# debbiemarkslab/BEAR

Measured on AMD Instinct MI355X. Metric: k-mer contexts/sec (DM-marginal+grad h), k=13, higher is better.
Workload: dtype f64

## Files before the change

bear_amd/csrc/bear_cnn.hip:

```cpp
#include "bear_host.h"
#include "kernels_cnn.h"

int cnn_ws_setup(bear_ws *) { return allow_dynamic_lds({BEAR_KFN(cnn_backward_head_kernel)}, cnh_lds_bytes()); }

#ifdef CNN_STAMPS
extern "C" int bear_dbg_cnn_stamps(unsigned long long *host_out, int reset) {
  if (host_out) HIP_TRY(hipMemcpyFromSymbol(host_out, HIP_SYMBOL(cnn_stamp_sums), sizeof(unsigned long long) * 8));
  if (reset) {
    unsigned long long z[8] = {0, 0, 0, 0, 0, 0, 0, 0};
    HIP_TRY(hipMemcpyToSymbol(HIP_SYMBOL(cnn_stamp_sums), z, sizeof(z)));
  }
  return BEAR_OK;
}
#endif

static int cnn_forward_grid(const bear_ws *ws, uint64_t groups) {
  return grid_capped((groups + CNN_THREADS / 64 - 1) / (CNN_THREADS / 64), (uint64_t)ws->num_cu * 16);
}

static int cnn_check(const bear_ws *ws, int lag, int fw, int nf, int l1) {
  int st = check_ws(ws);
  if (st != BEAR_OK) return st;
  if (lag < 1 || lag > CNN_MAX_LAG || fw < 1 || fw > lag || nf != CNN_NF || l1 != CNN_L1) return BEAR_ERR_INVALID_ARG;
  return BEAR_OK;
// ... 13 lines not shown
  if (!kmer_code || !params || !prior || misaligned(t1_save) || misaligned8(prior)) return BEAR_ERR_INVALID_ARG;
  const cnn_dims D = cnn_make_dims(lag, filter_width);
  const size_t lds = sizeof(double) * (BEAR_EXPTAB_N + (size_t)filter_width * 6 * CNN_NF + (CNN_THREADS / 64) * CNN_FWD_SCRATCH);
  const int blocks = grid_capped((n_rows + CNN_THREADS - 1) / CNN_THREADS, (uint64_t)ws->num_cu * 16);
  hipLaunchKernelGGL(cnn_forward_kernel, dim3((unsigned)blocks), dim3(CNN_THREADS), lds, static_cast<hipStream_t>(stream),
                     reinterpret_cast<const unsigned long long *>(kmer_code), n_rows, D, params, prior, t1_save,
                     static_cast<const pln_tile *>(nullptr), static_cast<const uint16_t *>(nullptr), (n_rows + 63) / 64, cnn_all_positions(D));
  HIP_TRY(hipGetLastError());
  return BEAR_OK;
}

static int cnn_backward_grid(bear_ws *ws, const cnn_dims &D, uint64_t n_rows, int filter_width, int *waves_out, int *parts_out,
                             size_t *lds_out, uint64_t *blocks_out, hipStream_t s, int may_alloc) {
  const size_t fixed = sizeof(double) * (BEAR_EXPTAB_N + (size_t)filter_width * 6 * CNN_NF + (size_t)((D.total + 1) & ~1));
  const size_t lds2 = sizeof(double) * (cnnq_fixed_doubles(D) + (size_t)cnnq<2>::WAVES * cnnq<2>::WAVE_DOUBLES);
  const char *force = getenv("BEAR_CNN_BACKWARD");
  const bool det = bear_deterministic();
  int waves = det ? 1 : 4, parts = 0;
  while (waves > 1 && fixed + (size_t)waves * CNN_WAVE_DOUBLES * sizeof(double) > 160u * 1024u) waves >>= 1;
  size_t lds = fixed + (size_t)waves * CNN_WAVE_DOUBLES * sizeof(double);
  uint64_t per_block = (uint64_t)64 * waves;
  if (lds2 <= 160u * 1024u && !(force && force[0] == '1')) {
    parts = 1;
    waves = det ? 1 : cnnq<2>::WAVES;
    lds = sizeof(double) * (cnnq_fixed_doubles(D) + (size_t)waves * cnnq<2>::WAVE_DOUBLES);
    per_block = (uint64_t)cnnq<2>::TILE * waves;
  }
  if (lds > 160u * 1024u) return BEAR_ERR_INVALID_ARG;
  const uint64_t blocks = (uint64_t)grid_capped((n_rows + per_block - 1) / per_block, (uint64_t)ws->num_cu);
  const size_t need = (size_t)blocks * D.total;
  if (ws->cnn_partials_cap < need) {
    if (!may_alloc) return BEAR_ERR_INVALID_ARG;
    HIP_TRY(hipStreamSynchronize(s));
    if (ws->cnn_partials) (void)hipFree(ws->cnn_partials);
    ws->cnn_partials = nullptr;
    ws->cnn_partials_cap = 0;
    HIP_TRY(hipMalloc(&ws->cnn_partials, sizeof(double) * need));
    ws->cnn_partials_cap = need;
  }
  *waves_out = waves;
  *parts_out = parts;
  *lds_out = lds;
  *blocks_out = blocks;
  return BEAR_OK;
}

static int launch_cnn_backward(bear_ws *ws, const cnn_dims &D, const uint64_t *kmer_code, uint64_t n_rows, int filter_width,
                               const double *params, const double *t1_save, const double *prior, const double *grad_prior,
                               double *grad_params, hipStream_t s, int may_alloc, const bear_plan *live_plan = nullptr) {
  int waves = 0, parts = 0;
  size_t lds = 0;
  uint64_t blocks = 0;
  int st = cnn_backward_grid(ws, D, n_rows, filter_width, &waves, &parts, &lds, &blocks, s, may_alloc);
  if (st != BEAR_OK) return st;
  const bool parts2 = parts != 0;
  const void *fn = parts2 ? reinterpret_cast<const void *>(cnn_backward_parts_kernel<2>) : reinterpret_cast<const void *>(cnn_backward_kernel);
  if (may_alloc) HIP_TRY(hipFuncSetAttribute(fn, hipFuncAttributeMaxDynamicSharedMemorySize, (int)lds));
  const unsigned long long *kc = reinterpret_cast<const unsigned long long *>(kmer_code);
  if (parts2) {
    const bool lists = live_plan && live_plan->live && live_plan->n_live_rows < n_rows;
    const uint64_t groups = lists ? live_plan->n_tiles : (n_rows + cnnq<2>::TILE - 1) / cnnq<2>::TILE;
    hipLaunchKernelGGL(cnn_backward_parts_kernel<2>, dim3((unsigned)blocks), dim3(64 * waves), lds, s, kc, n_rows, D, params, t1_save, prior,
                       grad_prior, ws->cnn_partials, lists ? live_plan->tiles : nullptr, lists ? live_plan->live : nullptr, groups,
                       cnn_all_positions(D));
  }
  else
    hipLaunchKernelGGL(cnn_backward_kernel, dim3((unsigned)blocks), dim3(64 * waves), lds, s, kc, n_rows, D, params, t1_save, prior,
                       grad_prior, ws->cnn_partials);
  hipLaunchKernelGGL(cnn_finalize_kernel, dim3((D.total + 3) / 4), dim3(256), 0, s, ws->cnn_partials, (int)blocks, D.total, grad_params);
  HIP_TRY(hipGetLastError());
  return BEAR_OK;
}

int bear_cnn_backward_f64(bear_ws *ws, const uint64_t *kmer_code, uint64_t n_rows, int lag, int filter_width, int num_filters,
                          int layer1_width, const double *params, const double *t1_save, const double *prior,
                          const double *grad_prior, double *grad_params, void *stream) {
  int st = cnn_check(ws, lag, filter_width, num_filters, layer1_width);
  if (st != BEAR_OK) return st;
  if (!params || !grad_params) return BEAR_ERR_INVALID_ARG;
  if (n_rows && (!kmer_code || !t1_save || !prior || !grad_prior || misaligned(t1_save))) return BEAR_ERR_INVALID_ARG;
  const cnn_dims D = cnn_make_dims(lag, filter_width);
  return launch_cnn_backward(ws, D, kmer_code, n_rows, filter_width, params, t1_save, prior, grad_prior, grad_params,
                             static_cast<hipStream_t>(stream), 1);
}

int bear_cnn_reserve(bear_ws *ws, uint64_t n_rows, int lag, int filter_width, int num_filters, int layer1_width) {
  int st = cnn_check(ws, lag, filter_width, num_filters, layer1_width);
  if (st != BEAR_OK) return st;
  const cnn_dims D = cnn_make_dims(lag, filter_width);
  int waves = 0, parts = 0;
  size_t lds = 0;
  uint64_t blocks = 0;
  st = cnn_backward_grid(ws, D, n_rows, filter_width, &waves, &parts, &lds, &blocks, nullptr, 1);
  if (st != BEAR_OK) return st;
  HIP_TRY(hipFuncSetAttribute(parts ? reinterpret_cast<const void *>(cnn_backward_parts_kernel<2>)
                                                      : reinterpret_cast<const void *>(cnn_backward_kernel),
                              hipFuncAttributeMaxDynamicSharedMemorySize, (int)lds));
  return BEAR_OK;
}

static int cnn_forward_levels(bear_ws *ws, const bear_plan *plan, const cnn_dims &D, const uint64_t *kmer_code, uint64_t n_rows,
                              const double *params, double *prior, double *t1_buf, hipStream_t s);
static cnn_level_io cnn_level_positions(const bear_plan *plan, const cnn_dims &D, int k) {
  const int K = plan->n_cnn_levels;
  const int L = k == 0 ? D.lag : plan->cnn_levels[k - 1].letters;
  cnn_level_io io = cnn_all_positions(D);
  io.p_hi = L - D.fw + 1;
  io.p_lo = k == K ? 0 : plan->cnn_levels[k].letters - D.fw + 1;
  io.head = k == 0;
  io.p_hi -= plan->n_cnn_win[k];
  return io;
}
static cnn_level_io cnn_window_positions(const cnn_dims &D, const bear_window_dev &wt) {
  cnn_level_io io = cnn_all_positions(D);
  io.p_lo = wt.pos;
  io.p_hi = io.p_lo + 1;
  io.head = 0;
  return io;
}
static void cnn_level_sources(const bear_plan *plan, int k, cnn_level_io &io) {
  if (k < plan->n_cnn_levels) {
    io.t1_parent = plan->cnn_levels[k].rows;
    io.parent = plan->cnn_levels[k].parent_of_below;
  }
  io.n_win = plan->n_cnn_win[k];
  for (int q = 0; q < plan->n_cnn_win[k]; ++q) {
    io.win_rows[q] = plan->cnn_win[k][q].rows;
    io.win_row_of[q] = plan->cnn_win[k][q].row_of_context;
  }
}
static bool cnn_parts_form_forced_off() {
  const char *force = getenv("BEAR_CNN_BACKWARD");
  return force && force[0] == '1';
}
static int cnn_train_reduce_levels(bear_ws *ws, const bear_plan *plan, const cnn_dims &D, const uint64_t *kmer_code, uint64_t n_rows,
                                   const double *theta, double *prior_buf, double *t1_buf, double *grad_rows_buf, double eps, int train_ar,
                                   double *packed, hipStream_t s) {
  const int K = plan->n_cnn_levels;
  const double *params = theta + 1;
  int bw_waves = 0, bw_parts = 0;
  size_t bw_lds = 0;
  uint64_t bw_blocks = 0;
  int st = cnn_backward_grid(ws, D, n_rows, D.fw, &bw_waves, &bw_parts, &bw_lds, &bw_blocks, s, 0);
  if (st != BEAR_OK) return st;
  if (!bw_parts) return BEAR_ERR_INVALID_ARG;
  auto level_codes = [&](int k) { return k == 0 ? reinterpret_cast<const unsigned long long *>(kmer_code) : plan->cnn_levels[k - 1].codes; };
  auto level_rows = [&](int k) { return k == 0 ? n_rows : plan->cnn_levels[k - 1].n; };
  auto level_table = [&](int k) { return k == 0 ? t1_buf : plan->cnn_levels[k - 1].rows; };
  auto level_io = [&](int k) { return cnn_level_positions(plan, D, k); };
  const cnn_level_io io0 = level_io(0);
  const bool recompute_t1 = io0.p_lo >= io0.p_hi && !getenv("BEAR_AMD_CNN_KEEP_T1");
  st = cnn_forward_levels(ws, plan, D, kmer_code, n_rows, params, prior_buf, recompute_t1 ? nullptr : t1_buf, s);
  if (st != BEAR_OK) return st;
  st = launch_prior_plan_grad(ws, plan, prior_buf, params_eps(eps), theta, train_ar, 1, packed, grad_rows_buf, s);
  if (st != BEAR_OK) return st;
  const uint64_t per_block = (uint64_t)cnnq<2>::TILE * (uint64_t)bw_waves;
  bool first_launch = true;
  auto backward = [&](const unsigned long long *codes, uint64_t n, const double *t1_in, cnn_level_io io) {
    const uint64_t blocks = first_launch ? bw_blocks : (uint64_t)grid_capped((n + per_block - 1) / per_block, bw_blocks);
    io.accumulate = first_launch ? 0 : 1;
    first_launch = false;
    hipLaunchKernelGGL(cnn_backward_parts_kernel<2>, dim3((unsigned)blocks), dim3(64 * bw_waves), bw_lds, s, codes, n, D, params, t1_in, prior_buf,
                       grad_rows_buf, ws->cnn_partials, static_cast<const pln_tile *>(nullptr), static_cast<const uint16_t *>(nullptr),
                       (n + cnnq<2>::TILE - 1) / cnnq<2>::TILE, io);
  };
  for (int k = 0; k <= K; ++k) {
    cnn_level_io io = level_io(k);
    const uint64_t n = level_rows(k);
    const int W = plan->n_cnn_win[k];
    if (k > 0) {
      const int sb = grid_capped((n * (CNN_L1 / 2) + 255) / 256, (uint64_t)ws->num_cu * 32);
      hipLaunchKernelGGL(cnn_level_sum_kernel, dim3((unsigned)sb), dim3(256), 0, s, level_table(k - 1), plan->cnn_levels[k - 1].child_start,
                         n, level_table(k));
    }
    io.dT1 = (k == 0 && (K > 0 || W > 0)) ? t1_buf : (k > 0 ? level_table(k) : nullptr);
    if (k == 0 && recompute_t1) cnn_level_sources(plan, 0, io);
    if (k == 0 && io.p_lo >= io.p_hi && !getenv("BEAR_AMD_CNN_NO_HEAD_KERNEL")) {
      io.accumulate = first_launch ? 0 : 1;
      first_launch = false;
      hipLaunchKernelGGL(cnn_backward_head_kernel, dim3((unsigned)bw_blocks), dim3(CNH_WAVES * 64), cnh_lds_bytes(), s, n, D, params,
                         recompute_t1 ? static_cast<const double *>(nullptr) : t1_buf, prior_buf, grad_rows_buf, ws->cnn_partials, io);
    } else if (k == 0 || io.p_lo < io.p_hi) {
      backward(level_codes(k), n, (k == 0 && recompute_t1) ? static_cast<const double *>(nullptr) : t1_buf, io);
    }
    for (int q = 0; q < W; ++q) {
      const bear_window_dev &wt = plan->cnn_win[k][q];
      const int sb = grid_capped((wt.n + 3) / 4, (uint64_t)ws->num_cu * 8);
      hipLaunchKernelGGL(cnn_window_sum_kernel, dim3((unsigned)sb), dim3(256), 0, s, level_table(k), wt.perm, wt.child_start, wt.n, wt.rows);
      cnn_level_io wio = cnn_window_positions(D, wt);
      wio.dT1 = wt.rows;
      backward(wt.codes, wt.n, t1_buf, wio);
    }
  }
  hipLaunchKernelGGL(cnn_finalize_kernel, dim3((D.total + 3) / 4), dim3(256), 0, s, ws->cnn_partials, (int)bw_blocks, D.total, packed + 2);
  HIP_TRY(hipGetLastError());
  return BEAR_OK;
}

static void plan_drop_cnn_levels(bear_plan *plan) {
  for (int k = 0; k < plan->n_cnn_levels; ++k) {
    plan->bytes -= plan->cnn_levels[k].bytes;
    bear_level_free(&plan->cnn_levels[k]);
  }
  for (int k = 0; k <= CNN_MAX_LAG; ++k) {
    for (int q = 0; q < plan->n_cnn_win[k]; ++q) {
      plan->bytes -= plan->cnn_win[k][q].bytes;
      bear_window_free(&plan->cnn_win[k][q]);
    }
    plan->n_cnn_win[k] = 0;
  }
  plan->n_cnn_levels = 0;
  plan->n_cnn_windows = 0;
  plan->cnn_codes = nullptr;
}

int bear_plan_attach_cnn_levels(bear_plan *plan, const uint64_t *kmer_code, int lag, int filter_width, int *n_levels, void *stream) {
  if (n_levels) *n_levels = 0;
  if (!plan || plan->ncol != 5 || lag < 1 || lag > CNN_MAX_LAG || filter_width < 1 || filter_width > lag) return BEAR_ERR_INVALID_ARG;
  if (plan->n_rows && (!kmer_code || misaligned(kmer_code))) return BEAR_ERR_INVALID_ARG;
  hipStream_t s = static_cast<hipStream_t>(stream);
  HIP_TRY(hipStreamSynchronize(s));
  plan_drop_cnn_levels(plan);
  const cnn_dims D = cnn_make_dims(lag, filter_width);
  if (sizeof(double) * (cnnq_fixed_doubles(D) + (size_t)cnnq<2>::WAVES * cnnq<2>::WAVE_DOUBLES) > 160u * 1024u) return BEAR_OK;
  if (plan->n_rows < 2 || plan->n_live_rows != plan->n_rows) return BEAR_OK;
  const unsigned long long *below = reinterpret_cast<const unsigned long long *>(kmer_code);
  uint64_t n_below = plan->n_rows;
  int misses = 0;
  double keep_ratio = 0.6;
  if (const char *r = getenv("BEAR_AMD_CNN_LEVEL_RATIO")) keep_ratio = atof(r);
  for (int k = 1; k <= D.P - 1 && misses < 3; ++k) {
    bear_level_dev lv;
    const int st = bear_level_build(below, n_below, lag - k, &lv, s);
    if (st != BEAR_OK) {
      if (st == BEAR_ERR_HIP) g_last_hip_error = bear_count_last_hip_error();
      plan_drop_cnn_levels(plan);
      return st;
    }
    if ((double)lv.n > keep_ratio * (double)n_below) {
      bear_level_free(&lv);
      ++misses;
      continue;
    }
    misses = 0;
    lv.bytes = lv.n * (8 + 4 + 16 * 8) + 4 * n_below;
    plan->cnn_levels[plan->n_cnn_levels++] = lv;
    plan->bytes += lv.bytes;
    below = lv.codes;
    n_below = lv.n;
  }
  if (!getenv("BEAR_AMD_CNN_NO_WINDOWS")) {
    const int K = plan->n_cnn_levels;
    for (int k = 0; k <= K; ++k) {
      const unsigned long long *codes_k = k == 0 ? reinterpret_cast<const unsigned long long *>(kmer_code) : plan->cnn_levels[k - 1].codes;
      const uint64_t n_k = k == 0 ? plan->n_rows : plan->cnn_levels[k - 1].n;
      const int L = k == 0 ? lag : plan->cnn_levels[k - 1].letters;
      const int p_hi = L - filter_width + 1, p_lo = k == K ? 0 : plan->cnn_levels[k].letters - filter_width + 1;
      bear_window_dev built[CNN_MAX_WIN];
      int nb = 0;
      for (int p = p_hi - 1; p >= p_lo && nb < CNN_MAX_WIN && n_k >= 64; --p) {
        bear_window_dev wt;
        const int st = bear_window_build(codes_k, n_k, p, filter_width, &wt, s);
        if (st != BEAR_OK) {
          if (st == BEAR_ERR_HIP) g_last_hip_error = bear_count_last_hip_error();
          for (int q = 0; q < nb; ++q) bear_window_free(&built[q]);
          plan_drop_cnn_levels(plan);
          return st;
        }
        if (wt.n * 8 > n_k) {
          bear_window_free(&wt);
          break;
        }
        built[nb++] = wt;
      }
      for (int q = 0; q < nb; ++q) {
        plan->cnn_win[k][q] = built[nb - 1 - q];
        plan->bytes += plan->cnn_win[k][q].bytes;
      }
      plan->n_cnn_win[k] = nb;
      plan->n_cnn_windows += nb;
    }
  }
  if (plan->n_cnn_levels || plan->n_cnn_windows) {
    plan->cnn_codes = kmer_code;
    plan->cnn_lag = lag;
    plan->cnn_fw = filter_width;
  }
  if (n_levels) *n_levels = plan->n_cnn_levels;
  return BEAR_OK;
}

int bear_plan_cnn_window_rows(const bear_plan *plan, uint64_t *rows_out, int *pos_out, int *level_out, int capacity) {
  if (!plan || (capacity > 0 && !rows_out)) return BEAR_ERR_INVALID_ARG;
  int t = 0;
  for (int k = 0; k <= plan->n_cnn_levels; ++k)
    for (int q = 0; q < plan->n_cnn_win[k]; ++q, ++t)
      if (t < capacity) {
        rows_out[t] = plan->cnn_win[k][q].n;
        if (pos_out) pos_out[t] = plan->cnn_win[k][q].pos;
        if (level_out) level_out[t] = k;
      }
  return plan->n_cnn_windows;
}

int bear_plan_cnn_level_rows(const bear_plan *plan, uint64_t *rows_out, int *letters_out, int capacity) {
  if (!plan || (capacity > 0 && !rows_out)) return BEAR_ERR_INVALID_ARG;
  for (int k = 0; k < plan->n_cnn_levels && k < capacity; ++k) {
    rows_out[k] = plan->cnn_levels[k].n;
    if (letters_out) letters_out[k] = plan->cnn_levels[k].letters;
  }
  return plan->n_cnn_levels;
}

static int cnn_forward_levels(bear_ws *ws, const bear_plan *plan, const cnn_dims &D, const uint64_t *kmer_code, uint64_t n_rows,
                              const double *params, double *prior, double *t1_buf, hipStream_t s) {
  const int K = plan->n_cnn_levels;
  const size_t fwd_lds = sizeof(double) * (BEAR_EXPTAB_N + (size_t)D.fw * 6 * CNN_NF + (CNN_THREADS / 64) * CNN_FWD_SCRATCH);
  for (int k = K; k >= 0; --k) {
    for (int q = 0; q < plan->n_cnn_win[k]; ++q) {
      const bear_window_dev &wt = plan->cnn_win[k][q];
      const uint64_t groups = (wt.n + 63) / 64;
      const int blocks = cnn_forward_grid(ws, groups);
      hipLaunchKernelGGL(cnn_forward_kernel, dim3((unsigned)blocks), dim3(CNN_THREADS), fwd_lds, s, wt.codes, wt.n, D, params,
                         static_cast<double *>(nullptr), wt.rows, static_cast<const pln_tile *>(nullptr), static_cast<const uint16_t *>(nullptr),
                         groups, cnn_window_positions(D, wt));
    }
    cnn_level_io io = cnn_level_positions(plan, D, k);
    cnn_level_sources(plan, k, io);
    const uint64_t n = k == 0 ? n_rows : plan->cnn_levels[k - 1].n, groups = (n + 63) / 64;
    const int blocks = cnn_forward_grid(ws, groups);
    if (k == 0 && io.p_lo >= io.p_hi && !getenv("BEAR_AMD_CNN_NO_HEAD_KERNEL")) {
      const int hb = grid_capped((n + 32 * 16 - 1) / (32 * 16), (uint64_t)ws->num_cu * 2);
// ... 72 lines not shown
```

bear_amd/csrc/kernels_cnn.h:

```cpp
#pragma once
#include "bear_common.h"
#include "bear_levels.h"
#include "plan_common.h"

#define CNN_NF 30
#define CNN_L1 16
#define CNN_THREADS 256
#define CNN_LN_EPS 1e-5
#ifndef CNN_SHARED_RUNS
#define CNN_SHARED_RUNS 6
#endif
#ifndef CNN_FWD_RUNS
#define CNN_FWD_RUNS 4
#endif
#define CNN_FWD_KEEP 3
#define CNN_FWD_SCRATCH (96 + 16 * CNN_FWD_KEEP)

struct cnn_dims {
  int lag, fw, P;
  int oF, ob0, oW1, ob1, oW2, ob2, os0, os1, total;
};

static inline cnn_dims cnn_make_dims(int lag, int fw) {
  cnn_dims d;
  d.lag = lag;
  d.fw = fw;
  d.P = lag - fw + 1;
  d.oF = 0;
  d.ob0 = d.oF + fw * 5 * CNN_NF;
  d.oW1 = d.ob0 + d.P * CNN_NF;
  d.ob1 = d.oW1 + d.P * CNN_NF * CNN_L1;
  d.oW2 = d.ob1 + CNN_L1;
  d.ob2 = d.oW2 + CNN_L1 * 5;
  d.os0 = d.ob2 + 5;
  d.os1 = d.os0 + d.P * CNN_NF;
  d.total = d.os1 + CNN_L1;
  return d;
}

struct cnn_level_io {
  int p_lo, p_hi;
  int head;
  int accumulate;
  const double *t1_parent;
  const uint32_t *parent;
  double *dT1;
  int n_win;
  const double *win_rows[CNN_MAX_WIN];
  const uint32_t *win_row_of[CNN_MAX_WIN];
};
static inline cnn_level_io cnn_all_positions(const cnn_dims &D) {
  cnn_level_io io;
  io.p_lo = 0;
  io.p_hi = D.P;
  io.head = 1;
  io.accumulate = 0;
  io.t1_parent = nullptr;
  io.parent = nullptr;
  io.dT1 = nullptr;
  io.n_win = 0;
  for (int q = 0; q < CNN_MAX_WIN; ++q) {
    io.win_rows[q] = nullptr;
    io.win_row_of[q] = nullptr;
  }
  return io;
}

__device__ __forceinline__ void cnn_stage_filters(double *Fs, const double *__restrict__ params, const cnn_dims &D) {
  for (int k = threadIdx.x; k < D.fw * 6 * CNN_NF; k += CNN_THREADS) {
    const int w = k / (6 * CNN_NF), r = k - w * 6 * CNN_NF, a = r / CNN_NF, f = r - a * CNN_NF;
    Fs[k] = a < 5 ? params[D.oF + (w * 5 + a) * CNN_NF + f] : 0.0;
  }
}

__device__ __forceinline__ double cnn_exp_neg(double z, const double *__restrict__ tab) {
  z = z > -700.0 ? z : -700.0;
  const double kf = __builtin_rint(z * 184.66496523378731);
  double r = __builtin_fma(kf, -0x1.62e42fee00000p-8, z);
  r = __builtin_fma(kf, -0x1.a39ef35793c76p-40, r);
  const int ki = (int)kf;
  const double t = tab[ki & (BEAR_EXPTAB_N - 1)];
  double p = __builtin_fma(r, 1.0 / 120.0, 1.0 / 24.0);
  p = __builtin_fma(r, p, 1.0 / 6.0);
  p = __builtin_fma(r, p, 0.5);
  p = __builtin_fma(r, p, 1.0);
  const double v = __builtin_fma(t, r * p, t);
  return __longlong_as_double(__double_as_longlong(v) + ((long long)(ki >> 7) << 52));
}

__device__ __forceinline__ double cnn_elu(double y, const double *exptab, double &deriv) {
  const double ex = cnn_exp_neg(y < 0.0 ? y : 0.0, exptab);
  deriv = y > 0.0 ? 1.0 : ex;
  return y > 0.0 ? y : ex - 1.0;
}

__device__ __forceinline__ double cnn_rsqrt(double v) {
  const double s = sqrt(v);
  return bear_rcp(s);
}

__device__ __forceinline__ double cnn_conv_norm(const double *Fs, unsigned long long code, int p, int fw, double (&x)[CNN_NF]) {
#pragma unroll
  for (int f = 0; f < CNN_NF; ++f) x[f] = 0.0;
  unsigned long long c = code >> (3 * p);
  for (int w = 0; w < fw; ++w) {
    const int a = (int)(c & 7ull);
    const double2 *row = reinterpret_cast<const double2 *>(Fs + (w * 6 + (a < 5 ? a : 5)) * CNN_NF);
    c >>= 3;
#pragma unroll
    for (int f2 = 0; f2 < CNN_NF / 2; ++f2) {
      const double2 v = row[f2];
      x[2 * f2] += v.x;
      x[2 * f2 + 1] += v.y;
    }
  }
  double m6[6] = {x[0], x[1], x[2], x[3], x[4], x[5]};
#pragma unroll
  for (int f = 6; f < CNN_NF; ++f) m6[f % 6] += x[f];
  const double mu = (((m6[0] + m6[1]) + (m6[2] + m6[3])) + (m6[4] + m6[5])) * (1.0 / CNN_NF);
  double v6[6] = {0.0, 0.0, 0.0, 0.0, 0.0, 0.0};
#pragma unroll
  for (int f = 0; f < CNN_NF; ++f) {
    x[f] -= mu;
    v6[f % 6] = __builtin_fma(x[f], x[f], v6[f % 6]);
  }
  const double var = ((v6[0] + v6[1]) + (v6[2] + v6[3])) + (v6[4] + v6[5]);
  const double r = cnn_rsqrt(var * (1.0 / CNN_NF) + CNN_LN_EPS);
#pragma unroll
  for (int f = 0; f < CNN_NF; ++f) x[f] *= r;
  return r;
}

__device__ __forceinline__ double cnn_layer1(const double (&t1)[CNN_L1], const double *__restrict__ params, const cnn_dims &D,
                                             const double *exptab, double (&n1)[CNN_L1], double (&e1)[CNN_L1],
                                             double (&d1)[CNN_L1]) {
  double mu = 0.0;
#pragma unroll
  for (int j = 0; j < CNN_L1; ++j) mu += t1[j];
  mu *= 1.0 / CNN_L1;
  double var = 0.0;
#pragma unroll
  for (int j = 0; j < CNN_L1; ++j) {
    n1[j] = t1[j] - mu;
    var = __builtin_fma(n1[j], n1[j], var);
  }
  const double r = cnn_rsqrt(var * (1.0 / CNN_L1) + CNN_LN_EPS);
#pragma unroll
  for (int j = 0; j < CNN_L1; ++j) {
    n1[j] *= r;
    e1[j] = cnn_elu(__builtin_fma(params[D.os1 + j], n1[j], params[D.ob1 + j]), exptab, d1[j]);
  }
  return r;
}

__device__ __forceinline__ double cnn_fwd_half_sum(double v) {
  auto dpp = [](double x, auto ctrl_tag) {
    constexpr int CTRL = decltype(ctrl_tag)::value;
    const long long q = __double_as_longlong(x);
    const int lo = __builtin_amdgcn_update_dpp(0, (int)(uint32_t)q, CTRL, 0xf, 0xf, false);
    const int hi = __builtin_amdgcn_update_dpp(0, (int)(uint32_t)(q >> 32), CTRL, 0xf, 0xf, false);
    return __longlong_as_double(((long long)hi << 32) | (uint32_t)lo);
  };
  v += dpp(v, std::integral_constant<int, 0xB1>{});
  v += dpp(v, std::integral_constant<int, 0x4E>{});
  v += dpp(v, std::integral_constant<int, 0x124>{});
  v += dpp(v, std::integral_constant<int, 0x128>{});
  const long long q = __double_as_longlong(v);
  const uint32_t lo = (uint32_t)q, hi = (uint32_t)(q >> 32);
  const auto a = __builtin_amdgcn_permlane16_swap(lo, lo, false, false);
  const auto c = __builtin_amdgcn_permlane16_swap(hi, hi, false, false);
  return __longlong_as_double(((long long)c[0] << 32) | a[0]) + __longlong_as_double(((long long)c[1] << 32) | a[1]);
}
__device__ __noinline__ void cnn_forward_shared_window2(const double *Fs, const double *exptab, double *Us, const double *__restrict__ s0_all,
                                                        const double *__restrict__ b0_all, const double *__restrict__ W1_all, int fw,
                                                        int p_a, unsigned long long win_a, int p_b, unsigned long long win_b, uint32_t lane) {
  const bool second = lane >= 32u;
  const uint32_t l32 = lane & 31u, f = l32 < CNN_NF ? l32 : CNN_NF - 1;
  const int p = second ? p_b : p_a;
  double xf = 0.0;
  unsigned long long c = second ? win_b : win_a;
  for (int w = 0; w < fw; w += 4) {
    double t4[4];
#pragma unroll
    for (int k = 0; k < 4; ++k) {
      const int a = (int)((c >> (3 * k)) & 7ull);
      t4[k] = Fs[(w + k < fw ? (w + k) * 6 + (a < 5 ? a : 5) : 5) * CNN_NF + f];
    }
    xf += (t4[0] + t4[1]) + (t4[2] + t4[3]);
    c >>= 12;
  }
  const bool in = l32 < CNN_NF;
  const double mu = cnn_fwd_half_sum(in ? xf : 0.0) * (1.0 / CNN_NF);
  const double d = xf - mu;
  const double r = cnn_rsqrt(cnn_fwd_half_sum(in ? d * d : 0.0) * (1.0 / CNN_NF) + CNN_LN_EPS);
  double dv;
  const double e = cnn_elu(__builtin_fma(s0_all[p * CNN_NF + (int)f], d * r, b0_all[p * CNN_NF + (int)f]), exptab, dv);
  double *Ue = Us + (second ? 32 : 0);
  if (in) Ue[l32] = e;
  if (l32 < CNN_L1) {
    const double *__restrict__ W1 = W1_all + p * CNN_NF * CNN_L1 + (int)l32;
    double u4[2] = {0.0, 0.0};
#pragma unroll 6
    for (int ff = 0; ff < CNN_NF; ++ff) u4[ff & 1] = __builtin_fma(Ue[ff], W1[ff * CNN_L1], u4[ff & 1]);
    Us[64 + (second ? 16 : 0) + l32] = u4[0] + u4[1];
  }
}

__global__ __launch_bounds__(CNN_THREADS, 4) void cnn_forward_kernel(const unsigned long long *__restrict__ codes, uint64_t n_rows,
                                                                   cnn_dims D, const double *__restrict__ params,
                                                                   double *__restrict__ prior, double *__restrict__ t1_save,
                                                                   const pln_tile *__restrict__ tiles, const uint16_t *__restrict__ live_lists,
                                                                   uint64_t n_groups, const cnn_level_io io) {
// ... 1043 lines not shown
        const double cs = cnnq_colsum<Q>(E, lane);
        if ((lane & 31u) < (uint32_t)CNN_NF) cnn_lds_add(G + D.os0 + p * CNN_NF + (int)(lane & 31u), cs);
      }
#pragma unroll
      for (int f = 0; f < FH; ++f) E[(h * FH + f) * CS + ctx] = dy[f];
      {
        const double cs = cnnq_colsum<Q>(E, lane);
        if ((lane & 31u) < (uint32_t)CNN_NF) cnn_lds_add(G + D.ob0 + p * CNN_NF + (int)(lane & 31u), cs);
      }
      CNN_STAMP(3)
      {
        unsigned long long c = code >> (3 * p);
        bool any_start = false;
        for (int w = w0; w < D.fw; ++w) any_start |= ((c >> (3 * w)) & 7ull) == 4ull;
#pragma unroll
        for (int f = 0; f < FH; ++f) {
          const double dc = (f >= FH - 2 && last) ? 0.0 : r0 * (dn[f] - ma0 - x[f] * ma1);
          if (f < FH - 2 || !last) E[(h * FH + f) * ES + ctx] = dc;
          dy[f] = dc;
        }
        if (w0 > 0) {
          const uint32_t cf = lane & 31u;
          const double2 *src = reinterpret_cast<const double2 *>(E + (cf < CNN_NF ? cf : 0u) * ES + (lane >> 5) * (TILE / 2));
          double s2[2] = {0.0, 0.0};
#pragma unroll
          for (int k = 0; k < TILE / 4; ++k) {
            const double2 v = src[k];
            s2[0] += v.x;
            s2[1] += v.y;
          }
          const double tot = cnnq_psum<Q>(s2[0] + s2[1]);
          unsigned long long cf1 = first >> (3 * p);
          for (int w = 0; w < w0; ++w) {
            const int a = (int)(cf1 & 7ull);
            if (a < 5 && lane < CNN_NF) cnn_lds_add(G + D.oF + (w * 5 + a) * CNN_NF + (int)lane, tot);
            cf1 >>= 3;
          }
        }
        if (any_start) {
          for (int w = w0; w < D.fw; ++w)
            if (((c >> (3 * w)) & 7ull) == 4ull) {
              double *gF = G + D.oF + (w * 5 + 4) * CNN_NF + h * FH;
#pragma unroll
              for (int f = 0; f < FH; ++f)
                if (f < FH - 2 || !last) cnn_lds_add(gF + f, dy[f]);
            }
        }
      }
      CNN_STAMP(4)
      auto d_filters = [&](auto nu_tag, int mt0) {
        constexpr int NU = decltype(nu_tag)::value;
        cnn_d4 acc[NU][2];
        int sh[NU];
        unsigned long long want[NU];
        bool row_ok[NU];
#pragma unroll
        for (int u = 0; u < NU; ++u) {
          acc[u][0] = cnn_d4{0.0, 0.0, 0.0, 0.0};
          acc[u][1] = cnn_d4{0.0, 0.0, 0.0, 0.0};
          const int row = (mt0 + u) * 16 + (int)lr, w = w0 + (row >> 2);
          want[u] = (unsigned long long)(row & 3);
          row_ok[u] = w < D.fw;
          sh[u] = row_ok[u] ? 3 * (p + w) : 0;
        }
        const bool col1_in = 16 + (int)lr < CNN_NF;
        const double *b1row = E + (col1_in ? 16 + (int)lr : 0) * ES + lq;
#pragma unroll
        for (int ks = 0; ks < KS; ++ks) {
          const unsigned long long cc = Cw[4 * ks + lq];
          const double b0v = E[lr * ES + 4 * ks + lq], b1v = col1_in ? b1row[4 * ks] : 0.0;
#pragma unroll
          for (int u = 0; u < NU; ++u) {
            const double a = (row_ok[u] && ((cc >> sh[u]) & 7ull) == want[u]) ? 1.0 : 0.0;
            acc[u][0] = __builtin_amdgcn_mfma_f64_16x16x4f64(a, b0v, acc[u][0], 0, 0, 0);
            acc[u][1] = __builtin_amdgcn_mfma_f64_16x16x4f64(a, b1v, acc[u][1], 0, 0, 0);
          }
        }
#pragma unroll
        for (int u = 0; u < NU; ++u)
#pragma unroll
          for (int r = 0; r < 4; ++r) {
            const int orow = (mt0 + u) * 16 + (int)lq + 4 * r, ow = w0 + (orow >> 2), oa = orow & 3;
            if (ow < D.fw) {
              double *gF = G + D.oF + (ow * 5 + oa) * CNN_NF;
              cnn_lds_add(gF + lr, acc[u][0][r]);
              if (lr < CNN_NF - 16) cnn_lds_add(gF + 16 + lr, acc[u][1][r]);
            }
          }
      };
      {
        const int n_mt_var = (4 * (D.fw - w0) + 15) / 16;
        int mt = 0;
        for (; mt + 1 < n_mt_var; mt += 2) d_filters(std::integral_constant<int, 2>{}, mt);
        if (mt < n_mt_var) d_filters(std::integral_constant<int, 1>{}, mt);
      }
      CNN_STAMP(5)
    }
    }
   }
  }
#ifndef CNN_NO_SHARED_BACKWARD
  {
    uint32_t ln = lane;
    asm volatile("" : "+v"(ln));
    for (int q = 0; q < C::CARRY_POS; ++q)
      if ((carry >> q) & 1u) flush_carried(q, ln);
    if (n_items) drain_items(ln);
  }
#endif
#ifdef CNN_STAMPS
  if (lane == 0)
    for (int k = 0; k < 8; ++k) atomicAdd(&cnn_stamp_sums[k], tph[k]);
#endif
  __syncthreads();
  for (int k = threadIdx.x; k < D.total; k += blockDim.x) {
    double *dst = partials + (size_t)blockIdx.x * D.total + k;
    *dst = io.accumulate ? *dst + G[k] : G[k];
  }
}

#define CNH_WAVES 12
#define CNH_NG (CNN_L1 * 5 + 5 + 2 * CNN_L1)
#define CNH_ES 36
#define CNH_WAVE_DOUBLES ((CNN_L1 + 5) * CNH_ES)
static inline size_t cnh_lds_bytes() { return sizeof(double) * (BEAR_EXPTAB_N + 2 * CNN_L1 + CNN_L1 * 5 + (size_t)CNH_WAVES * (CNH_WAVE_DOUBLES + CNH_NG)); }

__global__ __launch_bounds__(CNH_WAVES * 64) void cnn_backward_head_kernel(uint64_t n_rows, cnn_dims D, const double *__restrict__ params,
                                                                           const double *__restrict__ t1_save, const double *__restrict__ prior,
                                                                           const double *__restrict__ grad_prior, double *__restrict__ partials,
                                                                           const cnn_level_io io) {
  constexpr int TILE = 32, JH = CNN_L1 / 2, ES = CNH_ES, KS = TILE / 4;
  extern __shared__ __attribute__((aligned(16))) double cnn_lds[];
  double *exptab = cnn_lds, *Ps1 = exptab + BEAR_EXPTAB_N, *Pb1 = Ps1 + CNN_L1, *PW2 = Pb1 + CNN_L1;
  const uint32_t lane = threadIdx.x & 63u, n_waves = blockDim.x >> 6;
  const uint32_t wave = (uint32_t)__builtin_amdgcn_readfirstlane((int)(threadIdx.x >> 6));
  double *E = PW2 + CNN_L1 * 5 + wave * CNH_WAVE_DOUBLES;
  double *GW = PW2 + CNN_L1 * 5 + n_waves * CNH_WAVE_DOUBLES + wave * CNH_NG;
  for (int k = threadIdx.x; k < BEAR_EXPTAB_N; k += blockDim.x) exptab[k] = exp2((double)k * (1.0 / BEAR_EXPTAB_N));
  for (int k = threadIdx.x; k < CNN_L1; k += blockDim.x) {
    Ps1[k] = params[D.os1 + k];
    Pb1[k] = params[D.ob1 + k];
  }
  for (int k = threadIdx.x; k < CNN_L1 * 5; k += blockDim.x) PW2[k] = params[D.oW2 + k];
  __syncthreads();
  const uint32_t ctx = lane & (TILE - 1), h = lane / TILE, lq = lane >> 4, lr = lane & 15u;
  cnn_d4 acc_w2 = {0.0, 0.0, 0.0, 0.0};
  double acc_s1[JH], acc_b1[JH], acc_b2[5];
#pragma unroll
  for (int j = 0; j < JH; ++j) acc_s1[j] = acc_b1[j] = 0.0;
#pragma unroll
  for (int b = 0; b < 5; ++b) acc_b2[b] = 0.0;
  const uint64_t n_tiles = (n_rows + TILE - 1) / TILE;
  const uint64_t wave_id = (uint64_t)blockIdx.x * n_waves + wave, wave_cnt = (uint64_t)gridDim.x * n_waves;
  for (uint64_t g = n_tiles * wave_id / wave_cnt; g < n_tiles * (wave_id + 1) / wave_cnt; ++g) {
    const uint64_t i = g * TILE + ctx;
    const bool live = i < n_rows;
    double t1[JH], n1[JH], e1[JH], dy1[JH];
#pragma unroll
    for (int j = 0; j < JH; ++j) t1[j] = 0.0;
    double pr[5], gp[5];
#pragma unroll
    for (int b = 0; b < 5; ++b) {
      pr[b] = 0.2;
      gp[b] = 0.0;
    }
    if (live) {
      if (!t1_save) {
        if (io.t1_parent) {
          const double2 *src = reinterpret_cast<const double2 *>(io.t1_parent + (size_t)io.parent[i] * CNN_L1 + h * JH);
#pragma unroll
          for (int j = 0; j < JH / 2; ++j) {
            const double2 v = src[j];
            t1[2 * j] = v.x;
            t1[2 * j + 1] = v.y;
          }
        }
#pragma unroll
        for (int q = 0; q < CNN_MAX_WIN; ++q) {
          if (q < io.n_win) {
            const double2 *src = reinterpret_cast<const double2 *>(io.win_rows[q] + (size_t)io.win_row_of[q][i] * CNN_L1 + h * JH);
#pragma unroll
            for (int j = 0; j < JH / 2; ++j) {
              const double2 v = src[j];
              t1[2 * j] += v.x;
              t1[2 * j + 1] += v.y;
            }
          }
        }
      } else {
        const double2 *src = reinterpret_cast<const double2 *>(t1_save + i * CNN_L1 + h * JH);
#pragma unroll
        for (int j = 0; j < JH / 2; ++j) {
          const double2 v = src[j];
          t1[2 * j] = v.x;
          t1[2 * j + 1] = v.y;
        }
      }
#pragma unroll
      for (int b = 0; b < 5; ++b) {
        pr[b] = prior[i * 5 + b];
        gp[b] = grad_prior[i * 5 + b];
      }
    }
    double r1;
    {
      double mu = 0.0;
#pragma unroll
      for (int j = 0; j < JH; ++j) mu += t1[j];
      mu = cnnq_psum<2>(mu) * (1.0 / CNN_L1);
      double var = 0.0;
#pragma unroll
      for (int j = 0; j < JH; ++j) {
        n1[j] = t1[j] - mu;
        var = __builtin_fma(n1[j], n1[j], var);
      }
      r1 = cnn_rsqrt(cnnq_psum<2>(var) * (1.0 / CNN_L1) + CNN_LN_EPS);
    }
    double dz[5], sg = 0.0;
#pragma unroll
    for (int b = 0; b < 5; ++b) sg = __builtin_fma(pr[b], gp[b], sg);
#pragma unroll
    for (int b = 0; b < 5; ++b) dz[b] = pr[b] * (gp[b] - sg);
    {
      double ma = 0.0, mb = 0.0;
#pragma unroll
      for (int j = 0; j < JH; ++j) {
        n1[j] *= r1;
        double d1;
        e1[j] = cnn_elu(__builtin_fma(Ps1[h * JH + j], n1[j], Pb1[h * JH + j]), exptab, d1);
        double de = 0.0;
#pragma unroll
        for (int b = 0; b < 5; ++b) de = __builtin_fma(PW2[(h * JH + j) * 5 + b], dz[b], de);
        dy1[j] = de * d1;
        const double dn = dy1[j] * Ps1[h * JH + j];
        t1[j] = dn;
        ma += dn;
        mb = __builtin_fma(dn, n1[j], mb);
        acc_s1[j] = __builtin_fma(dy1[j], n1[j], acc_s1[j]);
        acc_b1[j] += dy1[j];
      }
      ma = cnnq_psum<2>(ma) * (1.0 / CNN_L1);
      mb = cnnq_psum<2>(mb) * (1.0 / CNN_L1);
#pragma unroll
      for (int j = 0; j < JH; ++j) t1[j] = r1 * (t1[j] - ma - n1[j] * mb);
    }
#pragma unroll
    for (int b = 0; b < 5; ++b) acc_b2[b] += dz[b];
#pragma unroll
    for (int j = 0; j < JH; ++j) E[(h * JH + j) * ES + ctx] = e1[j];
    if (h == 0) {
#pragma unroll
      for (int b = 0; b < 5; ++b) E[(CNN_L1 + b) * ES + ctx] = dz[b];
    }
    {
      const bool col_in = lr < 5u;
      const double *arow = E + lr * ES + lq, *brow = E + (CNN_L1 + (col_in ? lr : 0u)) * ES + lq;
#pragma unroll
      for (int ks = 0; ks < KS; ++ks) {
        const double a = arow[4 * ks], bv = col_in ? brow[4 * ks] : 0.0;
        acc_w2 = __builtin_amdgcn_mfma_f64_16x16x4f64(a, bv, acc_w2, 0, 0, 0);
      }
    }
    if (io.dT1 && live) {
      double2 *o = reinterpret_cast<double2 *>(io.dT1 + i * CNN_L1 + h * JH);
#pragma unroll
      for (int j = 0; j < JH / 2; ++j) o[j] = make_double2(t1[2 * j], t1[2 * j + 1]);
    }
  }
  if (lr < 5u) {
#pragma unroll
    for (int r = 0; r < 4; ++r) GW[((int)lq + 4 * r) * 5 + (int)lr] = acc_w2[r];
  }
#pragma unroll
  for (int b = 0; b < 5; ++b) {
    const double v = cnn_half_sum_all(acc_b2[b]);
    if (lane == 0u) GW[CNN_L1 * 5 + b] = v;
  }
#pragma unroll
  for (int j = 0; j < JH; ++j) {
    const double vs = cnn_half_sum_all(acc_s1[j]), vb = cnn_half_sum_all(acc_b1[j]);
    if (ctx == 0u) {
      GW[CNN_L1 * 5 + 5 + h * JH + j] = vs;
      GW[CNN_L1 * 5 + 5 + CNN_L1 + h * JH + j] = vb;
    }
  }
  __syncthreads();
  const double *G0 = PW2 + CNN_L1 * 5 + n_waves * CNH_WAVE_DOUBLES;
  double *row = partials + (size_t)blockIdx.x * D.total;
  if (!io.accumulate)
    for (int k = threadIdx.x; k < D.total; k += blockDim.x) row[k] = 0.0;
  __syncthreads();
  for (int k = threadIdx.x; k < CNH_NG; k += blockDim.x) {
    double v = 0.0;
    for (uint32_t w = 0; w < n_waves; ++w) v += G0[w * CNH_NG + k];
    const int dst = k < CNN_L1 * 5 ? D.oW2 + k : k < CNN_L1 * 5 + 5 ? D.ob2 + (k - CNN_L1 * 5)
                  : k < CNN_L1 * 5 + 5 + CNN_L1 ? D.os1 + (k - CNN_L1 * 5 - 5) : D.ob1 + (k - CNN_L1 * 5 - 5 - CNN_L1);
    row[dst] = io.accumulate ? row[dst] + v : v;
  }
}

__global__ __launch_bounds__(1024) void cnn_forward_head_kernel(uint64_t n_rows, cnn_dims D, const double *__restrict__ params,
                                                                double *__restrict__ prior, double *__restrict__ t1_save, const cnn_level_io io) {
  constexpr int TILE = 32, JH = CNN_L1 / 2;
  __shared__ double exptab[BEAR_EXPTAB_N], Ps1[CNN_L1], Pb1[CNN_L1], PW2[CNN_L1 * 5], Pb2[5];
  for (int k = threadIdx.x; k < BEAR_EXPTAB_N; k += blockDim.x) exptab[k] = exp2((double)k * (1.0 / BEAR_EXPTAB_N));
  for (int k = threadIdx.x; k < CNN_L1; k += blockDim.x) {
    Ps1[k] = params[D.os1 + k];
    Pb1[k] = params[D.ob1 + k];
  }
  for (int k = threadIdx.x; k < CNN_L1 * 5; k += blockDim.x) PW2[k] = params[D.oW2 + k];
  if (threadIdx.x < 5) Pb2[threadIdx.x] = params[D.ob2 + threadIdx.x];
  __syncthreads();
  const uint32_t lane = threadIdx.x & 63u, n_waves = blockDim.x >> 6;
  const uint32_t wave = (uint32_t)__builtin_amdgcn_readfirstlane((int)(threadIdx.x >> 6));
  const uint32_t ctx = lane & (TILE - 1), h = lane / TILE;
  const uint64_t n_tiles = (n_rows + TILE - 1) / TILE;
  const uint64_t wave_id = (uint64_t)blockIdx.x * n_waves + wave, wave_cnt = (uint64_t)gridDim.x * n_waves;
  for (uint64_t g = n_tiles * wave_id / wave_cnt; g < n_tiles * (wave_id + 1) / wave_cnt; ++g) {
    const uint64_t i = g * TILE + ctx;
    const bool live = i < n_rows;
    double t1[JH];
#pragma unroll
    for (int j = 0; j < JH; ++j) t1[j] = 0.0;
    if (live) {
      if (io.t1_parent) {
        const double2 *src = reinterpret_cast<const double2 *>(io.t1_parent + (size_t)io.parent[i] * CNN_L1 + h * JH);
#pragma unroll
        for (int j = 0; j < JH / 2; ++j) {
          const double2 v = src[j];
          t1[2 * j] = v.x;
          t1[2 * j + 1] = v.y;
        }
      }
#pragma unroll
      for (int q = 0; q < CNN_MAX_WIN; ++q) {
        if (q < io.n_win) {
          const double2 *src = reinterpret_cast<const double2 *>(io.win_rows[q] + (size_t)io.win_row_of[q][i] * CNN_L1 + h * JH);
#pragma unroll
          for (int j = 0; j < JH / 2; ++j) {
            const double2 v = src[j];
            t1[2 * j] += v.x;
            t1[2 * j + 1] += v.y;
          }
        }
      }
      if (t1_save) {
        double2 *o = reinterpret_cast<double2 *>(t1_save + i * CNN_L1 + h * JH);
#pragma unroll
        for (int j = 0; j < JH / 2; ++j) o[j] = make_double2(t1[2 * j], t1[2 * j + 1]);
      }
    }
    double mu = 0.0;
#pragma unroll
    for (int j = 0; j < JH; ++j) mu += t1[j];
    mu = cnnq_psum<2>(mu) * (1.0 / CNN_L1);
    double var = 0.0;
#pragma unroll
    for (int j = 0; j < JH; ++j) {
      t1[j] -= mu;
      var = __builtin_fma(t1[j], t1[j], var);
    }
    const double r1 = cnn_rsqrt(cnnq_psum<2>(var) * (1.0 / CNN_L1) + CNN_LN_EPS);
    double z[5] = {0.0, 0.0, 0.0, 0.0, 0.0};
#pragma unroll 2
    for (int j = 0; j < JH; ++j) {
      double dv;
      const double e = cnn_elu(__builtin_fma(Ps1[h * JH + j], t1[j] * r1, Pb1[h * JH + j]), exptab, dv);
#pragma unroll
      for (int b = 0; b < 5; ++b) z[b] = __builtin_fma(e, PW2[(h * JH + j) * 5 + b], z[b]);
    }
    double m = -INFINITY;
#pragma unroll
    for (int b = 0; b < 5; ++b) {
      z[b] = cnnq_psum<2>(z[b]) + Pb2[b];
      m = z[b] > m ? z[b] : m;
    }
    double tot = 0.0;
#pragma unroll
    for (int b = 0; b < 5; ++b) {
      z[b] = bear_exp_tab(z[b] - m, exptab);
      tot += z[b];
    }
    const double rt = bear_rcp(tot);
    if (live && h == 0) {
#pragma unroll
      for (int b = 0; b < 5; ++b) prior[i * 5 + b] = z[b] * rt;
    }
  }
}

__global__ __launch_bounds__(256) void cnn_level_sum_kernel(const double *__restrict__ child_rows, const uint32_t *__restrict__ child_start,
                                                            uint64_t n_rows, double *__restrict__ rows) {
  static_assert(CNN_L1 % 2 == 0, "rows of double2");
  constexpr uint32_t H = CNN_L1 / 2;
  const double2 *__restrict__ src = reinterpret_cast<const double2 *>(child_rows);
  double2 *__restrict__ dst = reinterpret_cast<double2 *>(rows);
  for (uint64_t t = (uint64_t)blockIdx.x * 256 + threadIdx.x; t < n_rows * H; t += (uint64_t)gridDim.x * 256) {
    const uint64_t u = t / H;
    const uint32_t j = (uint32_t)(t - u * H);
    const uint32_t c0 = child_start[u], c1 = child_start[u + 1];
    double2 s0 = {0.0, 0.0}, s1 = {0.0, 0.0};
    uint32_t c = c0;
    for (; c + 1 < c1; c += 2) {
      const double2 a = src[(size_t)c * H + j], b = src[(size_t)(c + 1) * H + j];
      s0.x += a.x;
      s0.y += a.y;
      s1.x += b.x;
      s1.y += b.y;
    }
    if (c < c1) {
      const double2 a = src[(size_t)c * H + j];
      s0.x += a.x;
      s0.y += a.y;
    }
    dst[t] = make_double2(s0.x + s1.x, s0.y + s1.y);
  }
}

__global__ __launch_bounds__(256) void cnn_window_sum_kernel(const double *__restrict__ child_rows, const uint32_t *__restrict__ perm,
// ... 48 lines not shown
```

Before: 138.7 billion.

## Fuse level-1 child summation into the CNN backward head kernel

The head backward kernel now sums the dT1 rows of each group of children straight into the parent level table, so the separate level-sum kernel launch for level 1 is skipped. Wave work ranges are snapped to parent group boundaries so that each parent's children stay inside one wave. Within a tile the kernel finds run starts with shuffles and ballots, then accumulates the runs serially through LDS and carries partial sums across tiles. This removes one kernel launch and one full re-read of the dT1 buffer. In exchange it adds serial per-run loops in LDS, possible load imbalance from the aligned ranges, and extra LDS traffic in the hot kernel.

```diff
diff --git a/bear_amd/csrc/bear_cnn.hip b/bear_amd/csrc/bear_cnn.hip
--- a/bear_amd/csrc/bear_cnn.hip
+++ b/bear_amd/csrc/bear_cnn.hip
@@ -189,6 +189,8 @@
   const bool recompute_t1 = io0.p_lo >= io0.p_hi && !getenv("BEAR_AMD_CNN_KEEP_T1");
   st = cnn_forward_levels(ws, plan, D, kmer_code, n_rows, params, prior_buf, recompute_t1 ? nullptr : t1_buf, s);
   if (st != BEAR_OK) return st;
+  const bool head_only = io0.p_lo >= io0.p_hi && !getenv("BEAR_AMD_CNN_NO_HEAD_KERNEL");
+  const bool fused_sum = head_only && K >= 1 && !getenv("BEAR_AMD_CNN_NO_FUSED_LEVEL_SUM");
   st = launch_prior_plan_grad(ws, plan, prior_buf, params_eps(eps), theta, train_ar, 1, packed, grad_rows_buf, s);
   if (st != BEAR_OK) return st;
   const uint64_t per_block = (uint64_t)cnnq<2>::TILE * (uint64_t)bw_waves;
@@ -205,16 +207,21 @@
     cnn_level_io io = level_io(k);
     const uint64_t n = level_rows(k);
     const int W = plan->n_cnn_win[k];
-    if (k > 0) {
+    if (k > 0 && !(k == 1 && fused_sum)) {
       const int sb = grid_capped((n * (CNN_L1 / 2) + 255) / 256, (uint64_t)ws->num_cu * 32);
       hipLaunchKernelGGL(cnn_level_sum_kernel, dim3((unsigned)sb), dim3(256), 0, s, level_table(k - 1), plan->cnn_levels[k - 1].child_start,
                          n, level_table(k));
     }
     io.dT1 = (k == 0 && (K > 0 || W > 0)) ? t1_buf : (k > 0 ? level_table(k) : nullptr);
     if (k == 0 && recompute_t1) cnn_level_sources(plan, 0, io);
-    if (k == 0 && io.p_lo >= io.p_hi && !getenv("BEAR_AMD_CNN_NO_HEAD_KERNEL")) {
+    if (k == 0 && head_only) {
       io.accumulate = first_launch ? 0 : 1;
       first_launch = false;
+      if (fused_sum) {
+        io.sum_parent = plan->cnn_levels[0].parent_of_below;
+        io.sum_child_start = plan->cnn_levels[0].child_start;
+        io.sum_rows = plan->cnn_levels[0].rows;
+      }
       hipLaunchKernelGGL(cnn_backward_head_kernel, dim3((unsigned)bw_blocks), dim3(CNH_WAVES * 64), cnh_lds_bytes(), s, n, D, params,
                          recompute_t1 ? static_cast<const double *>(nullptr) : t1_buf, prior_buf, grad_rows_buf, ws->cnn_partials, io);
     } else if (k == 0 || io.p_lo < io.p_hi) {
diff --git a/bear_amd/csrc/kernels_cnn.h b/bear_amd/csrc/kernels_cnn.h
--- a/bear_amd/csrc/kernels_cnn.h
+++ b/bear_amd/csrc/kernels_cnn.h
@@ -45,6 +45,9 @@
   const double *t1_parent;
   const uint32_t *parent;
   double *dT1;
+  const uint32_t *sum_parent;
+  const uint32_t *sum_child_start;
+  double *sum_rows;
   int n_win;
   const double *win_rows[CNN_MAX_WIN];
   const uint32_t *win_row_of[CNN_MAX_WIN];
@@ -58,6 +61,9 @@
   io.t1_parent = nullptr;
   io.parent = nullptr;
   io.dT1 = nullptr;
+  io.sum_parent = nullptr;
+  io.sum_child_start = nullptr;
+  io.sum_rows = nullptr;
   io.n_win = 0;
   for (int q = 0; q < CNN_MAX_WIN; ++q) {
     io.win_rows[q] = nullptr;
@@ -1407,9 +1413,20 @@
   for (int b = 0; b < 5; ++b) acc_b2[b] = 0.0;
   const uint64_t n_tiles = (n_rows + TILE - 1) / TILE;
   const uint64_t wave_id = (uint64_t)blockIdx.x * n_waves + wave, wave_cnt = (uint64_t)gridDim.x * n_waves;
-  for (uint64_t g = n_tiles * wave_id / wave_cnt; g < n_tiles * (wave_id + 1) / wave_cnt; ++g) {
-    const uint64_t i = g * TILE + ctx;
-    const bool live = i < n_rows;
+  const bool fuse = io.sum_parent != nullptr;
+  auto range_start = [&](uint64_t w) -> uint64_t {
+    const uint64_t g = n_tiles * w / wave_cnt;
+    if (g >= n_tiles) return n_rows;
+    return fuse ? (uint64_t)io.sum_child_start[io.sum_parent[g * TILE]] : g * TILE;
+  };
+  const uint64_t row_lo = range_start(wave_id), row_hi = range_start(wave_id + 1);
+  bool carried = false;
+  for (uint64_t base = row_lo; base < row_hi; base += TILE) {
+    const uint64_t i = base + ctx;
+    const bool live = i < row_hi;
+    uint32_t ps = 0;
+    uint32_t hoff = h * JH;
+    asm volatile("" : "+v"(hoff));
     double t1[JH], n1[JH], e1[JH], dy1[JH];
 #pragma unroll
     for (int j = 0; j < JH; ++j) t1[j] = 0.0;
@@ -1420,9 +1437,11 @@
       gp[b] = 0.0;
     }
     if (live) {
+      if (fuse) ps = io.sum_parent[i];
       if (!t1_save) {
         if (io.t1_parent) {
-          const double2 *src = reinterpret_cast<const double2 *>(io.t1_parent + (size_t)io.parent[i] * CNN_L1 + h * JH);
+          const uint32_t pi = io.parent == io.sum_parent ? ps : io.parent[i];
+          const double2 *src = reinterpret_cast<const double2 *>(io.t1_parent + ((size_t)pi * CNN_L1 + hoff));
 #pragma unroll
           for (int j = 0; j < JH / 2; ++j) {
             const double2 v = src[j];
@@ -1433,7 +1452,7 @@
 #pragma unroll
         for (int q = 0; q < CNN_MAX_WIN; ++q) {
           if (q < io.n_win) {
-            const double2 *src = reinterpret_cast<const double2 *>(io.win_rows[q] + (size_t)io.win_row_of[q][i] * CNN_L1 + h * JH);
+            const double2 *src = reinterpret_cast<const double2 *>(io.win_rows[q] + ((size_t)io.win_row_of[q][i] * CNN_L1 + hoff));
 #pragma unroll
             for (int j = 0; j < JH / 2; ++j) {
               const double2 v = src[j];
@@ -1443,7 +1462,7 @@
           }
         }
       } else {
-        const double2 *src = reinterpret_cast<const double2 *>(t1_save + i * CNN_L1 + h * JH);
+        const double2 *src = reinterpret_cast<const double2 *>(t1_save + (i * CNN_L1 + hoff));
 #pragma unroll
         for (int j = 0; j < JH / 2; ++j) {
           const double2 v = src[j];
@@ -1517,9 +1536,49 @@
       }
     }
     if (io.dT1 && live) {
-      double2 *o = reinterpret_cast<double2 *>(io.dT1 + i * CNN_L1 + h * JH);
+      double2 *o = reinterpret_cast<double2 *>(io.dT1 + (i * CNN_L1 + hoff));
 #pragma unroll
       for (int j = 0; j < JH / 2; ++j) o[j] = make_double2(t1[2 * j], t1[2 * j + 1]);
+    }
+    if (fuse) {
+#pragma unroll
+      for (int j = 0; j < JH; ++j) E[(h * JH + j) * ES + ctx] = t1[j];
+      const uint32_t cnt = row_hi - base < (uint64_t)TILE ? (uint32_t)(row_hi - base) : (uint32_t)TILE;
+      const uint32_t left = (uint32_t)__shfl_up((int)ps, 1, 64);
+      const bool is_start = live && (ctx == 0u || ps != left);
+      const uint32_t starts = (uint32_t)__builtin_amdgcn_ballot_w64(is_start);
+      bool open = false;
+      if (is_start) {
+        const uint32_t above = starts & ~((2u << ctx) - 1u);
+        const uint32_t end = above ? (uint32_t)__builtin_ctz(above) : cnt;
+        const double *col = E + h * JH * ES;
+        double s[JH];
+#pragma unroll
+        for (int j = 0; j < JH; ++j) s[j] = (ctx == 0u && carried) ? col[j * ES + TILE] : 0.0;
+        double nx[JH];
+#pragma unroll
+        for (int j = 0; j < JH; ++j) nx[j] = col[j * ES + ctx];
+        for (uint32_t c = ctx; c < end; ++c) {
+          double cur[JH];
+#pragma unroll
+          for (int j = 0; j < JH; ++j) {
+            cur[j] = nx[j];
+            nx[j] = col[j * ES + c + 1];
+          }
+#pragma unroll
+          for (int j = 0; j < JH; ++j) s[j] += cur[j];
+        }
+        open = end == cnt && (uint64_t)io.sum_child_start[ps + 1] > base + cnt;
+        if (open) {
+#pragma unroll
+          for (int j = 0; j < JH; ++j) E[(h * JH + j) * ES + TILE] = s[j];
+        } else {
+          double2 *o = reinterpret_cast<double2 *>(io.sum_rows + ((size_t)ps * CNN_L1 + hoff));
+#pragma unroll
+          for (int j = 0; j < JH / 2; ++j) o[j] = make_double2(s[2 * j], s[2 * j + 1]);
+        }
+      }
+      carried = __builtin_amdgcn_ballot_w64(open) != 0ull;
     }
   }
   if (lr < 5u) {
```

After: 138.8 billion (median of 2 runs). About the same (+0.0%).
